# invokermyself/ICP-4DRadar

Hardware: AMD Instinct MI355X
Metric: scan-pair registrations/sec (8k-pt clouds, 20 ICP iters) at 1/2/4/8 GPU (higher is better)
Workload: dtype fp32; 1 GPU; C3/C4: 1024 independent pairs per GPU, 8192/8192-pt scans, 20 ICP iterations (fixed) + fitness pass, exact NN (kd-block pruned), PCL numerics (bit-exact float restatement); pairs_per_gpu=1024, points=8192, parallelism=1 GPU

## Files before the change

### icp-4dradar_amd/csrc/icp4r_batch.hpp

```cpp
#pragma once

#include <hip/hip_runtime.h>

#include <vector>

#include "icp4r_host.hpp"
#include "icp4r_internal.hpp"

namespace icp4r_pipe {

struct Plan {
    int q;
    bool packed;
    int splits;
    bool pruned;
    bool lds;
    bool cache;
    int leaf;
    int chunk_sb;
    int chunks;
    bool tile;
    int max_m;
    int tile_run;
    bool solo;
    int64_t blocks;
};

enum PlanOpt : int {
    kOptNnQ, kOptLeaf, kOptChunkSb, kOptNnLds, kOptNnCache, kOptNnTile, kOptTileRun, kOptSolo, kOptXpad,
    kOptPhaseTicks, kOptKd, kOptMortonMwg, kOptPart, kOptSrcOrder, kOptFuseSeed, kOptTileOwn, kOptTileDefer,
    kOptGroups, kOptSearchCuDiv, kOptFuseTest, kOptFuseOrder, kOptSumsTail, kOptWideUpdate, kOptGatherPadded,
    kOptGicpCovBrute, kOptFoldKeys, kOptGicpSpec, kOptGicpGrid, kOptGicpKnnLanes, kOptResUpdate, kOptHeldUpdate,
    kOptFitXform, kOptCounters, kOptStageSel, kOptLazyX, kNumPlanOpts
};
static_assert(kNumPlanOpts <= 64, "icp4r_ctx::plan_set is a 64-bit mask");
extern const char* const kPlanOptNames[kNumPlanOpts];
int opt(const icp4r_ctx* ctx, PlanOpt k, int dflt);

Plan make_plan(const icp4r_ctx* ctx, int npairs, int max_n, int max_m, int nn_mode = ICP4R_NN_AUTO,
               bool allow_lds = true, bool registration = false);
int make_kparams(const icp4r_params* p, icp4r::KParams* kp);
int setup_work(icp4r_ctx* ctx, const Plan& pl, int npairs, int max_n, int max_m, bool corr, hipStream_t st,
               icp4r::WorkArgs& w);
int nn_pass(icp4r_ctx* ctx, const Plan& pl, const icp4r::PairArgs& a, const icp4r::WorkArgs& w, int npairs, int max_n,
            int fitness_pass, int first, hipStream_t st, int ncu = 0, int test_fused = 0, int pass = -1,
            int ordered = 0, int pending = 0);
int next_event(std::vector<icp4r_host::EventPair>& v, size_t& used, icp4r_host::EventPair** out);

// ... 2 lines not shown
```

### icp-4dradar_amd/csrc/icp4r_capi.cpp

```cpp
#include <dlfcn.h>
#include <float.h>
#include <hip/hip_runtime.h>
#include <math.h>
#include <stdlib.h>
#include <string.h>

#include <algorithm>
#include <cstdarg>
#include <cstdio>
#include <string>
#include <utility>
#include <vector>

#include "icp4r/icp4r.h"
#include "icp4r_batch.hpp"
#include "icp4r_host.hpp"
#include "icp4r_internal.hpp"

using namespace icp4r;

namespace icp4r_host {

thread_local std::string g_last_error;

// ... 41 lines not shown
    return api;
}

}

using icp4r_host::DevBuf;
using icp4r_host::EventPair;
using icp4r_host::check_cloud;
using icp4r_host::fail;
using icp4r_host::pack_host;

namespace icp4r_pipe {

constexpr size_t kCountBytes = (size_t)kCountSlots * kCountStride * sizeof(uint64_t);

constexpr int kNumCounters = 8;
int read_counters(icp4r_ctx* ctx, uint64_t (&out)[kNumCounters]) {
    for (int k = 0; k < kNumCounters; ++k) out[k] = 0;
    HIP_TRY(hipSetDevice(ctx->device));
    HIP_TRY(hipDeviceSynchronize());
    if (!ctx->evals.p) return ICP4R_OK;
    std::vector<uint64_t> v((size_t)kCountSlots * kCountStride);
    HIP_TRY(hipMemcpy(v.data(), ctx->evals.p, kCountBytes, hipMemcpyDeviceToHost));
    for (int s = 0; s < kCountSlots; ++s)
        for (int k = 0; k < kNumCounters; ++k) out[k] += v[(size_t)s * kCountStride + k];
    return ICP4R_OK;
}

const char* const kPlanOptNames[kNumPlanOpts] = {
    "nn_q", "leaf", "chunk_sb", "nn_lds", "nn_cache", "nn_tile", "tile_run", "solo", "xpad",
    "phase_ticks", "kd", "morton_mwg", "part", "src_order", "fuse_seed", "tile_own", "tile_defer",
    "groups", "search_cu_div", "fuse_test", "fuse_order", "sums_tail", "wide_update", "gather_padded",
    "gicp_cov_brute", "fold_keys", "gicp_spec", "gicp_grid", "gicp_knn_lanes", "res_update",
    "held_update", "fit_xform", "counters", "stage_sel", "lazy_x"};

int opt(const icp4r_ctx* ctx, PlanOpt k, int dflt) {
    return (ctx && (ctx->plan_set >> k & 1ull)) ? ctx->plan_val[k] : dflt;
}

Plan make_plan(const icp4r_ctx* ctx, int npairs, int max_n, int max_m, int nn_mode, bool allow_lds,
               bool registration) {
    Plan pl;
    pl.pruned = nn_mode == ICP4R_NN_PRUNED || (nn_mode == ICP4R_NN_AUTO && max_m >= kPrunedMinM);
    pl.packed = false;
    pl.lds = false;
    pl.cache = false;
    pl.splits = 1;
    pl.leaf = 0;
    pl.chunk_sb = 64;
// ... 385 lines not shown
    const int iters = max_iterations > 0 ? max_iterations : 1;
    const bool fuse = pl.lds && pl.cache && pcl && opt(ctx, kOptFuseTest, 1) != 0;
    const bool ford = fuse && opt(ctx, kOptFuseOrder, 1) != 0;
    for (int g = 0; g < groups; ++g)
        wg[g].sums_tail = (fuse && a.kp.huber_delta == INFINITY && a.kp.max_d2 >= FLT_MAX && !a.kp.need_mse &&
                           opt(ctx, kOptSumsTail, 0) != 0)
                              ? 1
                              : 0;
    for (int g = 0; g < groups; ++g)
        wg[g].res_update = (fuse && pcl && mn <= kResMaxN && !wg[g].sums_tail && a.kp.huber_delta == INFINITY &&
                             a.kp.max_d2 >= FLT_MAX && opt(ctx, kOptResUpdate, kDefaultResUpdate) != 0)
                                ? 1
                                : 0;
    const bool lazy = fuse && !wg[0].sums_tail && !wg[0].res_update && opt(ctx, kOptLazyX, kDefaultLazyX) != 0;
    for (int g = 0; g < groups; ++g) wg[g].lazy_x = lazy ? 1 : 0;
    auto silent_tail = [&](int it) { return lazy && it >= 0 && it + 1 < iters && ((iters - 2 - it) & 1) != 0; };
    const bool kev = ctx->kernel_timing;
    const bool wide = pcl && !fuse && npairs <= ctx->ncu && opt(ctx, kOptWideUpdate, 1) != 0;
    for (int g = 0; g < groups; ++g)
        wg[g].held_update = (wide && mn <= kHeldMaxN && opt(ctx, kOptHeldUpdate, kDefaultHeldUpdate) != 0) ? 1 : 0;
    if (wide && pl.tile && !pl.lds && w.corr && (pl.chunks > 1 || !w.tile_own) && opt(ctx, kOptFoldKeys, 1) != 0)
        for (int g = 0; g < groups; ++g) wg[g].fold_keys = 1;
    char pass_name[48];
    for (int it = 0; it < iters; ++it) {
        snprintf(pass_name, sizeof(pass_name), "icp4r ICP pass %d", it + 1);
        icp4r_host::Range pass_range(pass_name);
        for (int g = 0; g < groups; ++g) {
            const int ncu_g = search_cu > 0 ? search_cu : ctx->ncu;
            if ((rc = nn_pass(ctx, pl, ag[g], wg[g], gn[g], mn, 0, it == 0, gs[g], search_cu, fuse && it > 0, it,
                              ford && it > 0, silent_tail(it - 1) ? 1 : 0)))
// ... 473 lines not shown
    return -1;
}
}

int icp4r_set_plan_option(icp4r_ctx* ctx, const char* name, int32_t value) {
    if (!ctx) return fail(ICP4R_E_INVALID, "ctx is NULL");
    const int k = plan_opt_index(name);
    if (k < 0) return fail(ICP4R_E_INVALID, "unknown plan option '%s'", name ? name : "(null)");
    if (k == kOptGroups && (value < 1 || value > kMaxGroups))
        return fail(ICP4R_E_INVALID,
                    "plan option groups = %d: 1..%d (a fourth pair group shares a hardware queue with the third, "
                    "and its kernels serialise)",
                    value, kMaxGroups);
    if (k == kOptXpad && (value < 0 || value > 1 << 20)) return fail(ICP4R_E_INVALID, "plan option xpad = %d", value);
    if (k == kOptSearchCuDiv && value < 0) return fail(ICP4R_E_INVALID, "plan option search_cu_div = %d", value);
    ctx->plan_val[k] = value;
    ctx->plan_set |= 1ull << k;
    return ICP4R_OK;
}

int icp4r_get_plan_option(const icp4r_ctx* ctx, const char* name, int32_t* value, int32_t* is_set) {
    if (!ctx || !value) return fail(ICP4R_E_INVALID, "NULL argument");
    const int k = plan_opt_index(name);
    if (k < 0) return fail(ICP4R_E_INVALID, "unknown plan option '%s'", name ? name : "(null)");
    const bool set = (ctx->plan_set >> k) & 1ull;
    *value = set ? ctx->plan_val[k] : INT32_MIN;
    if (!set) {
        static const int32_t dflt[kNumPlanOpts] = {
            0 , kDefaultLeaf, 0 , -1 , 1, 1, 0 ,
            -1 , 0, 0, 3, 1, kDefaultPartSize, -1 , 1, 1, 1, kDefaultGroups,
            0 , 1, 1, 0, 1, 0, 0, 1, kGicpSpec, kGicpGrid,
            0 , kDefaultResUpdate, kDefaultHeldUpdate, 1, 0, kDefaultStageSel, kDefaultLazyX};
        *value = dflt[k];
    }
    if (is_set) *is_set = set ? 1 : 0;
    return ICP4R_OK;
}

int icp4r_reset_plan_options(icp4r_ctx* ctx) {
    if (!ctx) return fail(ICP4R_E_INVALID, "ctx is NULL");
    ctx->plan_set = 0;
    return ICP4R_OK;
}

int icp4r_plan(const icp4r_ctx* ctx, int32_t npairs, int32_t max_src_n, int32_t max_tgt_n, int32_t nn_mode,
               int32_t numerics, icp4r_plan_info* out) {
    if (npairs <= 0 || max_src_n < 0 || max_tgt_n < 0 || !out) return fail(ICP4R_E_INVALID, "bad shape");
// ... 39 lines not shown

int icp4r_nn_stats(icp4r_ctx* ctx, icp4r_nn_stats_t* out) {
    if (!ctx || !out) return fail(ICP4R_E_INVALID, "NULL argument");
    uint64_t v[kNumCounters];
    int rc = read_counters(ctx, v);
    if (rc) return rc;
    memset(out, 0, sizeof(*out));
    out->evaluations = v[0];
    out->box_tests = v[1];
    out->cache_hits = v[2];
    out->cache_tested = v[3];
    out->records_written_by_test = v[4];
    out->tested_in_update = v[5];
    out->hits_in_update = v[6];
    out->second_chance_hits = v[7];
    return ICP4R_OK;
}

int icp4r__debug_ticks(icp4r_ctx* ctx, uint64_t* out, int32_t k) {
    if (!ctx || !out || k <= 0 || (size_t)k * sizeof(uint64_t) > ctx->ticks.cap) return fail(ICP4R_E_INVALID, "bad arguments");
    if (!ctx->ticks.p) return fail(ICP4R_E_INVALID, "phase ticks not enabled (plan option phase_ticks = 1)");
    HIP_TRY(hipSetDevice(ctx->device));
    HIP_TRY(hipDeviceSynchronize());
    HIP_TRY(hipMemcpy(out, ctx->ticks.p, (size_t)k * sizeof(uint64_t), hipMemcpyDeviceToHost));
    return ICP4R_OK;
}

int icp4r__test_rot_f32(icp4r_ctx* ctx, const float* sigma, float* R, int32_t k) {
    if (!ctx || !sigma || !R || k <= 0) return fail(ICP4R_E_INVALID, "bad arguments");
    HIP_TRY(hipSetDevice(ctx->device));
// ... 11 lines not shown
```

### icp-4dradar_amd/csrc/icp4r_frame.hip

```cpp
#include "icp4r_fold.hpp"

namespace icp4r {

template <int kInitWG>
__global__ __launch_bounds__(kInitWG) void init_kernel(PairArgs a, WorkArgs w) {
    __shared__ float Tg[16];
    __shared__ int ident;
    const int p = xcd_remap(blockIdx.x, gridDim.x);
    const int tid = threadIdx.x;
    const int n = a.src_n[p], m = a.tgt_n[p];
    const float4* src = a.src + a.src_off[p];
    const float4* tgt = a.tgt + a.tgt_off[p];
    PairState& st = w.state[p];
    if (tid < 16) Tg[tid] = a.guess ? a.guess[(int64_t)p * 16 + tid] : ((tid % 5 == 0) ? 1.0f : 0.0f);
    __syncthreads();
    if (tid == 0) {
        bool id = true;
        for (int k = 0; k < 16; ++k) id = id && (Tg[k] == ((k % 5 == 0) ? 1.0f : 0.0f));
        ident = id ? 1 : 0;
    }
    __syncthreads();
    constexpr int kInitPer = 4;
    float4* X = w.X + (int64_t)p * w.x_stride;
    const bool id = ident != 0;
// ... 53 lines not shown
        for (int k = tid; k < w.need_stride; k += kInitWG) gneed[k] = 0u;
    }
    if (tid == 0 && w.miss_cnt) w.miss_cnt[p] = 0;
    if (tid < 4 && p == 0 && w.plist_n) w.plist_n[tid] = 0;
    bad = __syncthreads_or(bad);
    big = __syncthreads_or(big);
    if (tid == 0) {
        mat4_identity(st.T_inc);
        st.prev_mse = DBL_MAX;
        st.similar = 0;
        st.conv_state = 0;
        st.iterations = 0;
        st.ncorr = 0;
        st.sums_ok = big ? -1 : 0;
        st.pending = 0;
        const bool too_big = n > w.x_stride || (w.leaf > 0 && m > w.t_stride);
        if (m <= 0 || bad || too_big) {
            mat4_identity(st.final_T);
            st.phase = kPhaseInvalid;
            st.status = too_big ? kStatusInvalid : m <= 0 ? kStatusEmpty : kStatusNonFinite;
        } else {
            for (int k = 0; k < 16; ++k) st.final_T[k] = Tg[k];
            st.phase = kPhaseActive;
            st.status = 0;
        }
    }
}

constexpr int kPrepWG = 256;
constexpr int kPrepRecs = 1024;
// ... 227 lines not shown
```

### icp-4dradar_amd/csrc/icp4r_internal.hpp

```cpp
#pragma once

#include <hip/hip_runtime.h>
#include <stdint.h>

#include "icp4r/icp4r.h"
#include "icp4r/icp4r_ego.h"
#include "icp4r/icp4r_gicp.h"
#include "icp4r_math.hpp"

namespace icp4r {

constexpr int kNNWG = 256;
constexpr int kMaxQ = 16;
constexpr int kDefaultQ = 4;
constexpr int kDefaultPrunedQ = 2;
constexpr int kDefaultLeaf = 16;
constexpr int kMaxGroups = 3;
constexpr int kDefaultGroups = 2;
constexpr int kDefaultStageSel = 32;
constexpr int kDefaultPartSize = 2048;
constexpr int kFoldChunk = 1024;
constexpr int kSuper = 8;
constexpr int kPrunedMinM = 512;
constexpr int kCacheMaxN = 16384;
// ... 29 lines not shown
};

struct PairArgs {
    const float4* src;
    const float4* tgt;
    const int64_t* src_off;
    const int32_t* src_n;
    const int64_t* tgt_off;
    const int32_t* tgt_n;
    const float* guess;
    float4* aligned;
    Result* results;
    KParams kp;
};

struct PairState {
    float T_inc[16];
    float final_T[16];
    double prev_mse;
    int32_t similar;
    int32_t conv_state;
    int32_t iterations;
    int32_t phase;
    int32_t status;
    int32_t ncorr;
    float sum_s[3];
    int32_t sums_ok;
    float T_pend[16];
    int32_t pending;
};

using NNKey = uint64_t;
__host__ __device__ inline float key_d2(NNKey k) {
    union {
        uint32_t u;
        float f;
    } c;
    c.u = (uint32_t)(k >> 32);
    return c.f;
}
__host__ __device__ inline int32_t key_idx(NNKey k) { return (int32_t)(uint32_t)k; }

struct WorkArgs {
    float4* X;
// ... 15 lines not shown
    int32_t* tinv;
    float4* tbox;
    float4* sbox;
    int32_t* sperm;
    int64_t t_stride, b_stride, sb_stride;
    float4* corr;
    float* nn_u;
    int32_t tile_own;
    int32_t defer_xform;
    int32_t sums_tail;
    int32_t fold_keys;
    int32_t res_update;
    int32_t held_update;
    int32_t fit_xform;
    int32_t lazy_x;
    float4* nn_t;
    float4* sq;
    uint2* sm;
    float4* qv;
    uint2* qm;
    uint32_t* need;
    int64_t need_stride;
    int32_t* miss_cnt;
    int32_t* plist;
    int32_t* plist_n;
    int32_t* queue;
    int32_t* owork;
    int32_t part_size;
    int32_t stage_sel;
    unsigned long long* evals;
// ... 13 lines not shown
                            int max_n, int fitness_pass, int first, hipStream_t st);
hipError_t launch_nn_tile(const PairArgs& a, const WorkArgs& w, int npairs, int max_n, int max_m, int fitness_pass,
                          int first, int qrun, hipStream_t st, hipEvent_t tile_start = nullptr, hipEvent_t tile_stop = nullptr);
struct NNLdsEvents {
    hipEvent_t test_start = nullptr, test_stop = nullptr, search_start = nullptr, search_stop = nullptr;
};
hipError_t launch_nn_lds(const PairArgs& a, const WorkArgs& w, int npairs, int max_n, int fitness_pass, int first,
                         int ncu, hipStream_t st, const NNLdsEvents& ev, int test_fused = 0, int ordered = 0,
                         int pending = 0);
constexpr int kLdsMaxTargets = 8192;
constexpr int kLdsMinPairs = 256;
constexpr int kLdsMaxSources = 1 << 14;
constexpr int kResMaxN = 8192;
constexpr int kDefaultResUpdate = 0;
constexpr int kDefaultLazyX = 1;
constexpr int kHeldMaxN = 10 * 896;
constexpr int kHeldSmallN = 3 * 704;
constexpr int kDefaultHeldUpdate = 1;
constexpr int kSoloMaxN = 1024;
hipError_t launch_update(const PairArgs& a, const WorkArgs& w, int npairs, int max_n, bool need_corr,
                         hipStream_t st, int tail_test = 0,
                         int order_ncu = 0,
                         bool wide = false,
                         int silent = 0,
                         int pending = 0);
hipError_t launch_solo(const PairArgs& a, const WorkArgs& w, int npairs, int max_n, int iters, hipStream_t st);
hipError_t launch_fitness_prep(const PairArgs& a, const WorkArgs& w, int npairs, hipStream_t st, int test = 0);
hipError_t launch_finish(const PairArgs& a, const WorkArgs& w, int npairs, hipStream_t st);
hipError_t launch_rot_f32(const float* sigma, float* R, int k, hipStream_t st);

// ... 179 lines not shown
```

### icp-4dradar_amd/csrc/icp4r_kernels.hip

```cpp
#include "icp4r_fold.hpp"

namespace icp4r {

template <int Q>
__device__ __forceinline__ void nn_sweep(const float (&x)[Q], const float (&y)[Q], const float (&z)[Q],
                                         const float4* tgt_generic, int j0, int j1, float (&best)[Q],
                                         int (&bi)[Q]) {
    const cv4f_ptr tgt = as_const(tgt_generic);
#pragma unroll
    for (int q = 0; q < Q; ++q) {
        best[q] = INFINITY;
        bi[q] = j0;
    }
    const int last = j1 - 1;
    for (int j = j0; j < j1; j += 4) {
        const v4f c[4] = {tgt[j], tgt[min(j + 1, last)], tgt[min(j + 2, last)], tgt[min(j + 3, last)]};
#pragma unroll
        for (int t = 0; t < 4; ++t) {
#pragma unroll
            for (int q = 0; q < Q; ++q) {
                const float d = l2_simple(x[q], y[q], z[q], c[t].x, c[t].y, c[t].z);
                if (d < best[q]) {
                    best[q] = d;
                    bi[q] = j + t;
// ... 1485 lines not shown
}
__device__ __forceinline__ void wave_exact_total(uint64_t& S, int& E) {
    int e = E;
#pragma unroll
    for (int off = 32; off > 0; off >>= 1) e = min(e, __shfl_xor(e, off, 64));
    uint64_t t = E == INT_MAX ? 0 : exact_rescale(S, E - e);
#pragma unroll
    for (int off = 32; off > 0; off >>= 1) t = min(t + __shfl_xor(t, off, 64), kExactSat);
    S = t;
    E = e;
}

constexpr int kSliceGroup = 14;
constexpr int kFillBatch = 2;

template <int WG, int CH, int ROW>
__device__ __forceinline__ void fold_pass_a(const KParams& kp, const FoldIn& f, float (*buf)[9][ROW], float* res,
                                            int32_t* wcnt, SolveShared& s, const float* sums = nullptr) {
    const int tid = threadIdx.x, lane = tid & 63, wave = tid >> 6;
    const bool weighted = kp.huber_delta < INFINITY;
    auto rec = [&](int i, float4& r0, float4& r1) {
        if (f.C) {
            r0 = f.C[2 * i];
            r1 = f.C[2 * i + 1];
        } else {
            r0 = f.X[i];
            r1 = f.NT[i];
        }
    };
    auto rec_fix = [&](float4& r0, float4& r1) {
        if (!f.C) {
            if (f.Tp) pend_pt(f.Tp, r0);
            const float d2 = l2_simple(r0.x, r0.y, r0.z, r1.x, r1.y, r1.z);
// ... 15 lines not shown
#pragma unroll
            for (int e = 0; e < kPerA; ++e) {
                const int i = base + min(tid - fill0 + e * nf, len - 1);
                r[e][0] = f.X[i];
                ti[e] = (uint32_t)key_idx(f.K[i]);
            }
#pragma unroll
            for (int e = 0; e < kPerA; ++e) r[e][1] = f.TG[ti[e]];
            return;
        }
#pragma unroll
        for (int e = 0; e < kPerA; ++e) {
            const int i = base + min(tid - fill0 + e * nf, len - 1);
            if (sums)
                r[e][1] = f.NT[i];
            else
                rec(i, r[e][0], r[e][1]);
        }
    };
    auto store_a = [&](int c, float4 (&r)[kPerA][2]) __attribute__((always_inline)) {
        float(*b)[ROW] = buf[c & 1];
        const int base = c * CH, len = min(CH, n - base), nf = WG - fill0;
#pragma unroll
        for (int e = 0; e < kPerA; ++e) {
            const int o = tid - fill0 + e * nf;
            if (o >= len) break;
            if (sums) {
#pragma unroll
                for (int k = 0; k < 3; ++k) b[3 + k][o] = (&r[e][1].x)[k];
                b[6][o] = 1.0f;
                ++cnt;
                continue;
            }
            rec_fix(r[e][0], r[e][1]);
            const float d2 = r[e][1].w;
            if (f.Cw) {
                f.Cw[2 * (base + o)] = r[e][0];
                f.Cw[2 * (base + o) + 1] = r[e][1];
            }
            const float sv[6] = {r[e][0].x, r[e][0].y, r[e][0].z, r[e][1].x, r[e][1].y, r[e][1].z};
            float v[6], wt = 0.0f, dd = 0.0f;
#pragma unroll
            for (int k = 0; k < 6; ++k) v[k] = ident;
            if (!(d2 > kp.max_d2)) {
                wt = r[e][0].w;
#pragma unroll
                for (int k = 0; k < 6; ++k) v[k] = weighted ? wt * sv[k] : sv[k];
                dd = d2;
                ++cnt;
            }
#pragma unroll
            for (int k = 0; k < 6; ++k) b[k][o] = v[k];
            b[6][o] = wt;
            reinterpret_cast<double*>(b[7])[o] = (double)dd;
        }
    };
    float acc = (lane < 6) ? ident : 0.0f;
    double dacc = 0.0;
    const int wv = __builtin_amdgcn_readfirstlane(wave);
    if (wv == 0) {
        const int lane0 = sums ? 3 : 0;
        fold_prio(true);
        for (int c = 0; c < nch; ++c) {
            __syncthreads();
            if (lane >= lane0 && lane < 7) acc = fold_seq<float>(buf[c & 1][lane], min(CH, n - c * CH), acc);
        }
        fold_prio(false);
    } else if (wv * 64 < fill0) {
        uint64_t xs = 0;
        int xe = INT_MAX;
        for (int c = 0; c < nch; ++c) {
            __syncthreads();
            const double* dv = reinterpret_cast<const double*>(buf[c & 1][7]);
            const int len = min(CH, n - c * CH);
            for (int o = lane; o < len; o += 64) lane_exact_add(dv[o], xs, xe);
        }
        wave_exact_total(xs, xe);
        dacc = xs >= kExactSat ? -1.0 : (xe == INT_MAX ? 0.0 : ldexp((double)xs, xe));
    } else {
        if (nch > 0) {
            float4 r[kPerA][2];
            load_a(0, r);
            store_a(0, r);
        }
        for (int c = 0; c < nch; ++c) {
            __syncthreads();
            if (c + 1 < nch) {
                float4 r[kPerA][2];
                load_a(c + 1, r);
                store_a(c + 1, r);
            }
        }
    }
    cnt = wave_sumi(cnt);
    if (lane == 0) wcnt[wave] = cnt;
    if (wave == 0 && lane < 7) res[lane] = (sums && lane < 3) ? sums[lane] : acc;
    if (wave == 1 && lane == 0) s.mse_sum = dacc;
    __syncthreads();
    if (tid == 0) {
        int total = 0;
        for (int k = 0; k < (WG / 64); ++k) total += wcnt[k];
        s.mom[0] = (double)total;
        const float one_over_n = 1.0f / res[6];
        s.one_over_n = one_over_n;
        for (int k = 0; k < 6; ++k) s.mean[k] = res[k] * one_over_n;
    }
    __syncthreads();
    if (mse && s.mse_sum < 0.0) {
        dacc = 0.0;
        if (wv == 0) {
            for (int c = 0; c < nch; ++c) __syncthreads();
        } else if (wv * 64 < fill0) {
            for (int c = 0; c < nch; ++c) {
                __syncthreads();
                if (lane == 0) dacc = fold_seq_d(reinterpret_cast<const double*>(buf[c & 1][7]), min(CH, n - c * CH), dacc);
            }
// ... 430 lines not shown
        wt[0] = __builtin_amdgcn_s_memrealtime();
        wt[5] = (uint64_t)(uint32_t)__builtin_amdgcn_s_getreg(4 | (31 << 11)) |
                ((uint64_t)(uint32_t)__builtin_amdgcn_s_getreg(20 | (31 << 11)) << 32);
    }
#define WG_TICK(k) \
    if (wt) wt[k] = __builtin_amdgcn_s_memrealtime()
#else
#define WG_TICK(k)
#endif
    const bool lazy = w.lazy_x && w.nn_u && !C && !w.sums_tail;
    const float* Tp = PEND ? st.T_pend : nullptr;
    FoldIn fin{C, Xp, NT, n};
    fin.Tp = Tp;
    const bool sums_tail = w.sums_tail && tail_test && w.nn_u && !C;
    const bool use_sums = sums_tail && uload(&st.sums_ok) == 1;
    fold_pass_a<kFoldWG, kFoldChunkP, kFoldRow>(kp, fin, sh.buf, sh.res, sh.cnt, sh.s, use_sums ? st.sum_s : nullptr);
    if (use_sums && tid == 0) st.sums_ok = 0;
    if (ticks) w.ticks[1] = __builtin_amdgcn_s_memrealtime();
    WG_TICK(1);
    fold_pass_b<kFoldWG, kFoldChunkP, kFoldRow, false>(kp, fin, sh.buf, sh.s);
    if (ticks) w.ticks[2] = __builtin_amdgcn_s_memrealtime();
    WG_TICK(2);
    const bool tail = tail_test && w.nn_u;
    int nwork = 0;
    TailFirst<kTailPer> tf;
    uint32_t* need = reinterpret_cast<uint32_t*>(&sh.buf[0][0][0]);
    if (tail) {
        if (!sums_tail && n > 0) tail_prefetch<kFoldWG, kTailPer>(w, p, n, tf);
        for (int k = tid; k < ((n + 31) >> 5); k += kFoldWG) need[k] = 0u;
        if (tid == 0) sh.mcount = 0;
    }
    if (tid == 0) solve_pair<kNumericsPCL>(sh.s, st, kp);
// ... 22 lines not shown
            float* stg = reinterpret_cast<float*>(&sh.buf[0][0][0]) + (2 * 9 * kFoldRow - 2 * kSumBuf);
            nwork = pair_cache_test<kFoldWG, kSumPer, false, true>(
                a, w, p, n, T, need, pre, lv, lm, kFoldRecsSums, &sh.mcount, sh.cnt, false, stamp, nullptr, stg,
                st.sum_s, &st.sums_ok);
        } else {
            const bool quiet = lazy && silent && !Tp;
            nwork = pair_cache_test<kFoldWG, kTailPer, false>(a, w, p, n, T, need, pre, lv, lm, kFoldRecs,
                                                                    &sh.mcount, sh.cnt, false, stamp, &tf, nullptr,
                                                                    nullptr, nullptr, Tp, quiet);
            if (quiet) {
                if (tid < 16) st.T_pend[tid] = sh.s.T_inc[tid];
                if (tid == 0) st.pending = 1;
            } else if (Tp && tid == 0) {
                st.pending = 0;
            }
        }
    }
    if (ticks) w.ticks[4] = __builtin_amdgcn_s_memrealtime();
    WG_TICK(4);
    return nwork;
}

template <bool PEND>
__global__ __launch_bounds__(kFoldWG, 4) void fold_update_kernel(PairArgs a, WorkArgs w, int tail_test, int order_ncu,
                                                                             int silent) {
    __shared__ FoldShared sh;
    __shared__ OrderShared osh;
    __shared__ int32_t last;
    const int p = xcd_remap(blockIdx.x, gridDim.x);
    const int nwork = fold_update_pair<PEND>(a, w, tail_test, silent, p, sh);
// ... 1202 lines not shown
    }
#undef ICP4R_PR_CASE
    if (chunks > 1 && w.corr != nullptr && !fitness_pass)
        hipLaunchKernelGGL(corr_kernel, dim3((max_n + 255) / 256, npairs), dim3(256), 0, st, a, w);
    return hipGetLastError();
}

hipError_t launch_update(const PairArgs& a, const WorkArgs& w, int npairs, int max_n, bool need_corr, hipStream_t st,
                         int tail_test, int order_ncu, bool wide, int silent, int pending) {
    if (silent && pending) return hipErrorInvalidValue;
    if (order_ncu > 0 && (!tail_test || !w.owork || !w.plist || !w.plist_n || !w.nn_u || a.kp.numerics != kNumericsPCL))
        return hipErrorInvalidValue;
    if (w.lazy_x && (wide || need_corr || w.corr || w.res_update || w.sums_tail || !w.nn_u || !w.defer_xform ||
                     a.kp.numerics != kNumericsPCL))
        return hipErrorInvalidValue;
    if (a.kp.numerics == kNumericsPCL) {
        if (need_corr)
            hipLaunchKernelGGL(corr_kernel, dim3((max_n + 255) / 256, npairs), dim3(256), 0, st, a, w);
        if (wide && !tail_test && order_ncu <= 0 && w.held_update && max_n <= kHeldSmallN)
            hipLaunchKernelGGL((fold_update_held_kernel<3, true>), dim3(npairs), dim3(kWideWG), 0, st, a, w);
        else if (wide && !tail_test && order_ncu <= 0 && w.held_update && max_n <= kHeldMaxN)
            hipLaunchKernelGGL((fold_update_held_kernel<10, false>), dim3(npairs), dim3(kWideWG), 0, st, a, w);
        else if (wide && !tail_test && order_ncu <= 0)
            hipLaunchKernelGGL(fold_update_wide_kernel, dim3(npairs), dim3(kWideWG), 0, st, a, w);
        else if (w.res_update && !need_corr && !w.corr && max_n <= kResMaxN && w.nn_t && w.nn_u && w.defer_xform &&
                 a.kp.huber_delta == INFINITY && a.kp.max_d2 >= FLT_MAX &&
                 !w.sums_tail && (!tail_test || (w.sq && w.sm && w.need && w.miss_cnt)))
            hipLaunchKernelGGL(fold_update_res_kernel, dim3(npairs), dim3(kResWG), 0, st, a, w, tail_test, order_ncu);
        else if (w.lazy_x && pending)
            hipLaunchKernelGGL(fold_update_kernel<true>, dim3(npairs), dim3(kFoldWG), 0, st, a, w, tail_test, order_ncu, 0);
// ... 20 lines not shown
```

### icp-4dradar_amd/icp4r/__init__.py

```python
from __future__ import annotations

import ctypes as C
import os
import sys

import numpy as np

__all__ = [
    "ICP4RError", "Params", "Result", "Batch", "Context", "IterativeClosestPoint", "library_path", "load",
    "default_params", "NUMERICS_PCL", "NUMERICS_F64", "status_name", "EXPORTED_SYMBOLS", "Comm", "shard",
    "align_batch_multi",
]

HERE = os.path.dirname(os.path.abspath(__file__))
library_path = os.environ.get("ICP4R_LIBRARY") or os.path.join(HERE, "_lib", "libicp4r.so")

OK, E_INVALID, E_EMPTY, E_TOO_FEW_CORR, E_NONFINITE, E_HIP, E_RCCL, E_NOMEM, E_TOO_LARGE = 0, -1, -2, -3, -4, -5, -6, -7, -8
NUMERICS_PCL, NUMERICS_F64 = 0, 1
NO_DEVICE = -1
NN_AUTO, NN_BRUTE, NN_BRUTE_PACKED, NN_PRUNED = 0, 1, 2, 3
STAGE_NN, STAGE_NN_TEST, STAGE_UPDATE, STAGE_BATCH, STAGE_GICP_COV = 0, 1, 2, 3, 4
DBL_MAX = sys.float_info.max

_STATUS = {OK: "ICP4R_OK", E_INVALID: "ICP4R_E_INVALID", E_EMPTY: "ICP4R_E_EMPTY",
           E_TOO_FEW_CORR: "ICP4R_E_TOO_FEW_CORR", E_NONFINITE: "ICP4R_E_NONFINITE", E_HIP: "ICP4R_E_HIP",
           E_RCCL: "ICP4R_E_RCCL", E_NOMEM: "ICP4R_E_NOMEM", E_TOO_LARGE: "ICP4R_E_TOO_LARGE"}

EXPORTED_SYMBOLS = [
    "icp4r_version", "icp4r_abi_version", "icp4r_last_error", "icp4r_params_default", "icp4r_device_count",
    "icp4r_create", "icp4r_destroy", "icp4r_align", "icp4r_align_batch_device", "icp4r_align_batch_host",
    "icp4r_fitness", "icp4r_nearest", "icp4r_synchronize", "icp4r_kernel_time_ms", "icp4r_batch_time_ms",
    "icp4r_kernel_time_reset", "icp4r_set_kernel_timing", "icp4r_plan", "icp4r_nn_counters", "icp4r_nn_cache_hits", "icp4r_stage_time_ms",
    "icp4r_nn_stats", "icp4r_set_plan_option", "icp4r_get_plan_option", "icp4r_reset_plan_options",
]
PLAN_OPTIONS = (
    "nn_q", "leaf", "chunk_sb", "nn_lds", "nn_cache", "nn_tile", "tile_run", "solo", "xpad", "phase_ticks", "kd",
    "morton_mwg", "part", "src_order", "fuse_seed", "tile_own", "tile_defer", "groups", "search_cu_div",
    "fuse_test", "fuse_order", "sums_tail", "wide_update", "gather_padded", "gicp_cov_brute", "fold_keys", "gicp_spec", "gicp_grid", "gicp_knn_lanes", "res_update", "held_update", "fit_xform", "counters", "stage_sel",
    "lazy_x",
)
EGO_EXPORTED_SYMBOLS = [
    "icp4r_ego_params_default", "icp4r_radar_features", "icp4r_ego_velocity", "icp4r_ego_velocity_batch_device",
]
GATE_EXPORTED_SYMBOLS = [
    "icp4r_compact_by_mask_batch_device", "icp4r_static_clouds_batch_device", "icp4r_static_cloud",
    "icp4r_sequence_pairs", "icp4r_register_static_sequence", "icp4r_register_static_sequence_ex",
]
GICP_EXPORTED_SYMBOLS = [
    "icp4r_gicp_params_default", "icp4r_gicp_align", "icp4r_gicp_align_batch_device", "icp4r_gicp_covariances",
]
MULTI_EXPORTED_SYMBOLS = [
    "icp4r_shard", "icp4r_align_batch_multi", "icp4r_comm_unique_id", "icp4r_comm_create", "icp4r_comm_destroy",
    "icp4r_comm_rank", "icp4r_comm_check", "icp4r_gather_results", "icp4r_align_batch_sharded",
]
# ... 107 lines not shown
        "icp4r_align_batch_host": (C.c_int, [vp, vp, vp, vp, vp, vp, vp, i32, vp, C.POINTER(Params), vp]),
        "icp4r_fitness": (C.c_int, [vp, vp, i32, i32, vp, i32, i32, vp, C.c_double, C.POINTER(C.c_double)]),
        "icp4r_nearest": (C.c_int, [vp, vp, i32, i32, vp, i32, i32, vp, vp]),
        "icp4r_synchronize": (C.c_int, [vp, vp]),
        "icp4r_kernel_time_ms": (C.c_int, [vp, C.POINTER(C.c_double), C.POINTER(i32)]),
        "icp4r_batch_time_ms": (C.c_int, [vp, C.POINTER(C.c_double), C.POINTER(i32)]),
        "icp4r_kernel_time_reset": (C.c_int, [vp]),
        "icp4r_plan": (C.c_int, [vp, i32, i32, i32, i32, i32, C.POINTER(PlanInfo)]),
        "icp4r_set_plan_option": (C.c_int, [vp, C.c_char_p, i32]),
        "icp4r_get_plan_option": (C.c_int, [vp, C.c_char_p, C.POINTER(i32), C.POINTER(i32)]),
        "icp4r_reset_plan_options": (C.c_int, [vp]),
        "icp4r_nn_counters": (C.c_int, [vp, C.POINTER(C.c_uint64), C.POINTER(C.c_uint64)]),
        "icp4r_nn_cache_hits": (C.c_int, [vp, C.POINTER(C.c_uint64)]),
        "icp4r_stage_time_ms": (C.c_int, [vp, i32, C.POINTER(C.c_double), C.POINTER(i32)]),
        "icp4r_set_kernel_timing": (C.c_int, [vp, i32]),
        "icp4r_nn_stats": (C.c_int, [vp, C.POINTER(C.c_uint64 * 8)]),
        "icp4r_map_create": (C.c_int, [vp, C.POINTER(vp)]),
        "icp4r_map_destroy": (C.c_int, [vp]),
        "icp4r_map_build": (C.c_int, [vp, vp, i64, i32]),
        "icp4r_map_add_points": (C.c_int, [vp, vp, i64, i32, i32]),
        "icp4r_map_add_scan": (C.c_int, [vp, vp, i64, i32, vp, vp, vp]),
        "icp4r_map_size": (C.c_int, [vp, C.POINTER(i64)]),
        "icp4r_map_sector_search": (C.c_int, [vp, vp, C.c_float, C.c_float, vp, i64, C.POINTER(i64)]),
        "icp4r_map_sector_search_device": (C.c_int, [vp, vp, C.c_float, C.c_float, vp, vp, vp]),
        "icp4r_map_points_device": (C.c_int, [vp, C.POINTER(vp), C.POINTER(i64)]),
        "icp4r_map_time_ms": (C.c_int, [vp, C.POINTER(C.c_double), C.POINTER(i32)]),
        "icp4r_map_time_reset": (C.c_int, [vp]),
        "icp4r_map_add_points_downsample": (C.c_int, [vp, vp, i64, i32, C.c_float, C.POINTER(i64)]),
        "icp4r_map_delete_boxes": (C.c_int, [vp, vp, i32, C.POINTER(i64)]),
        "icp4r_map_box_search": (C.c_int, [vp, vp, vp, i64, C.POINTER(i64)]),
        "icp4r_map_radius_search": (C.c_int, [vp, vp, C.c_float, vp, i64, C.POINTER(i64)]),
# ... 166 lines not shown

    def stage_time_ms(self, stage: int) -> tuple[float, int]:
        ms, k = C.c_double(), C.c_int32()
        _check(self._lib.icp4r_stage_time_ms(self._h, stage, C.byref(ms), C.byref(k)), "icp4r_stage_time_ms")
        return ms.value, k.value

    def reset_timers(self):
        _check(self._lib.icp4r_kernel_time_reset(self._h), "icp4r_kernel_time_reset")

    def nn_counters(self) -> tuple[int, int]:
        v, t = C.c_uint64(), C.c_uint64()
        _check(self._lib.icp4r_nn_counters(self._h, C.byref(v), C.byref(t)), "icp4r_nn_counters")
        return v.value, t.value

    def nn_stats(self) -> dict:
        v = (C.c_uint64 * 8)()
        _check(self._lib.icp4r_nn_stats(self._h, C.byref(v)), "icp4r_nn_stats")
        keys = ("evaluations", "box_tests", "cache_hits", "cache_tested", "records_written_by_test",
                "tested_in_update", "hits_in_update", "second_chance_hits")
        return {k: int(v[i]) for i, k in enumerate(keys)}

    def nn_cache_hits(self) -> int:
        v = C.c_uint64()
        _check(self._lib.icp4r_nn_cache_hits(self._h, C.byref(v)), "icp4r_nn_cache_hits")
        return v.value

    def nn_evaluations(self) -> int:
        return self.nn_counters()[0]


def plan(npairs: int, max_src_n: int, max_tgt_n: int, nn_mode: int = NN_AUTO, numerics: int = NUMERICS_PCL,
         ctx: "Context | None" = None) -> dict:
    info = PlanInfo()
    _check(load().icp4r_plan(ctx.handle if ctx is not None else None, npairs, max_src_n, max_tgt_n, nn_mode, numerics,
# ... 193 lines not shown
```

### include/icp4r/icp4r.h

```cpp
#ifndef ICP4R_H
#define ICP4R_H

#include <stddef.h>
#include <stdint.h>

#ifdef __cplusplus
extern "C" {
#endif

#define ICP4R_ABI_VERSION 6

typedef enum icp4r_status {
    ICP4R_OK = 0,
    ICP4R_E_INVALID = -1,
    ICP4R_E_EMPTY = -2,
    ICP4R_E_TOO_FEW_CORR = -3,
    ICP4R_E_NONFINITE = -4,
    ICP4R_E_HIP = -5,
    ICP4R_E_RCCL = -6,
    ICP4R_E_NOMEM = -7,
    ICP4R_E_TOO_LARGE = -8
} icp4r_status;

typedef enum icp4r_convergence_state {
// ... 105 lines not shown
int icp4r_stage_time_ms(icp4r_ctx* ctx, int32_t stage, double* avg_ms, int32_t* launches);

int icp4r_nn_counters(icp4r_ctx* ctx, uint64_t* evaluations, uint64_t* box_tests);

int icp4r_nn_cache_hits(icp4r_ctx* ctx, uint64_t* hits);

typedef struct icp4r_nn_stats_t {
    uint64_t evaluations;
    uint64_t box_tests;
    uint64_t cache_hits;
    uint64_t cache_tested;
    uint64_t records_written_by_test;
    uint64_t tested_in_update;
    uint64_t hits_in_update;
    uint64_t second_chance_hits;
} icp4r_nn_stats_t;
int icp4r_nn_stats(icp4r_ctx* ctx, icp4r_nn_stats_t* out);

int icp4r_set_plan_option(icp4r_ctx* ctx, const char* name, int32_t value);
int icp4r_get_plan_option(const icp4r_ctx* ctx, const char* name, int32_t* value, int32_t* is_set);
int icp4r_reset_plan_options(icp4r_ctx* ctx);

typedef struct icp4r_plan_info {
    int32_t pruned;
    int32_t q;
    int32_t splits;
    int32_t leaf;
    int32_t lds;
    int32_t cache;
    int64_t nn_blocks;
// ... 14 lines not shown
```

Before: 157,000 pairs/s.

## Carry pass-A target sums across ICP iterations when correspondences are unchanged

Adds a carry_sums mode, on by default, that caches pass A's target-side sums and correspondence count in per-pair state. On the next iteration it checks whether any of the few changed correspondences actually moved, and if none did it folds only the source coordinates and reuses the cached target sums. This skips reading and folding the gathered target points in the update kernel. It adds a validation ballot, extra per-pair state, and a subtle correctness dependency on the change-tracking records.

```diff
diff --git a/icp-4dradar_amd/csrc/icp4r_batch.hpp b/icp-4dradar_amd/csrc/icp4r_batch.hpp
--- a/icp-4dradar_amd/csrc/icp4r_batch.hpp
+++ b/icp-4dradar_amd/csrc/icp4r_batch.hpp
@@ -31,7 +31,7 @@
     kOptPhaseTicks, kOptKd, kOptMortonMwg, kOptPart, kOptSrcOrder, kOptFuseSeed, kOptTileOwn, kOptTileDefer,
     kOptGroups, kOptSearchCuDiv, kOptFuseTest, kOptFuseOrder, kOptSumsTail, kOptWideUpdate, kOptGatherPadded,
     kOptGicpCovBrute, kOptFoldKeys, kOptGicpSpec, kOptGicpGrid, kOptGicpKnnLanes, kOptResUpdate, kOptHeldUpdate,
-    kOptFitXform, kOptCounters, kOptStageSel, kOptLazyX, kNumPlanOpts
+    kOptFitXform, kOptCounters, kOptStageSel, kOptLazyX, kOptCarrySums, kNumPlanOpts
 };
 static_assert(kNumPlanOpts <= 64, "icp4r_ctx::plan_set is a 64-bit mask");
 extern const char* const kPlanOptNames[kNumPlanOpts];
diff --git a/icp-4dradar_amd/csrc/icp4r_capi.cpp b/icp-4dradar_amd/csrc/icp4r_capi.cpp
--- a/icp-4dradar_amd/csrc/icp4r_capi.cpp
+++ b/icp-4dradar_amd/csrc/icp4r_capi.cpp
@@ -79,7 +79,7 @@
 
 constexpr size_t kCountBytes = (size_t)kCountSlots * kCountStride * sizeof(uint64_t);
 
-constexpr int kNumCounters = 8;
+constexpr int kNumCounters = 10;
 int read_counters(icp4r_ctx* ctx, uint64_t (&out)[kNumCounters]) {
     for (int k = 0; k < kNumCounters; ++k) out[k] = 0;
     HIP_TRY(hipSetDevice(ctx->device));
@@ -97,7 +97,7 @@
     "phase_ticks", "kd", "morton_mwg", "part", "src_order", "fuse_seed", "tile_own", "tile_defer",
     "groups", "search_cu_div", "fuse_test", "fuse_order", "sums_tail", "wide_update", "gather_padded",
     "gicp_cov_brute", "fold_keys", "gicp_spec", "gicp_grid", "gicp_knn_lanes", "res_update",
-    "held_update", "fit_xform", "counters", "stage_sel", "lazy_x"};
+    "held_update", "fit_xform", "counters", "stage_sel", "lazy_x", "carry_sums"};
 
 int opt(const icp4r_ctx* ctx, PlanOpt k, int dflt) {
     return (ctx && (ctx->plan_set >> k & 1ull)) ? ctx->plan_val[k] : dflt;
@@ -513,6 +513,9 @@
                                 : 0;
     const bool lazy = fuse && !wg[0].sums_tail && !wg[0].res_update && opt(ctx, kOptLazyX, kDefaultLazyX) != 0;
     for (int g = 0; g < groups; ++g) wg[g].lazy_x = lazy ? 1 : 0;
+    const bool carry = fuse && !wg[0].sums_tail && !wg[0].res_update && a.kp.huber_delta == INFINITY &&
+                       a.kp.max_d2 >= FLT_MAX && !a.kp.need_mse && opt(ctx, kOptCarrySums, kDefaultCarrySums) != 0;
+    for (int g = 0; g < groups; ++g) wg[g].carry_sums = carry ? 1 : 0;
     auto silent_tail = [&](int it) { return lazy && it >= 0 && it + 1 < iters && ((iters - 2 - it) & 1) != 0; };
     const bool kev = ctx->kernel_timing;
     const bool wide = pcl && !fuse && npairs <= ctx->ncu && opt(ctx, kOptWideUpdate, 1) != 0;
@@ -1016,6 +1019,8 @@
                     value, kMaxGroups);
     if (k == kOptXpad && (value < 0 || value > 1 << 20)) return fail(ICP4R_E_INVALID, "plan option xpad = %d", value);
     if (k == kOptSearchCuDiv && value < 0) return fail(ICP4R_E_INVALID, "plan option search_cu_div = %d", value);
+    if (k == kOptCarrySums && (value < 0 || value > 1))
+        return fail(ICP4R_E_INVALID, "plan option carry_sums = %d: 0 (off) or 1 (carry pass A's target sums)", value);
     ctx->plan_val[k] = value;
     ctx->plan_set |= 1ull << k;
     return ICP4R_OK;
@@ -1032,7 +1037,8 @@
             0 , kDefaultLeaf, 0 , -1 , 1, 1, 0 ,
             -1 , 0, 0, 3, 1, kDefaultPartSize, -1 , 1, 1, 1, kDefaultGroups,
             0 , 1, 1, 0, 1, 0, 0, 1, kGicpSpec, kGicpGrid,
-            0 , kDefaultResUpdate, kDefaultHeldUpdate, 1, 0, kDefaultStageSel, kDefaultLazyX};
+            0 , kDefaultResUpdate, kDefaultHeldUpdate, 1, 0, kDefaultStageSel, kDefaultLazyX,
+            kDefaultCarrySums};
         *value = dflt[k];
     }
     if (is_set) *is_set = set ? 1 : 0;
@@ -1102,6 +1108,8 @@
     out->tested_in_update = v[5];
     out->hits_in_update = v[6];
     out->second_chance_hits = v[7];
+    out->pass_a_carried_d = v[8];
+    out->pass_a_skipped = v[9];
     return ICP4R_OK;
 }
 
diff --git a/icp-4dradar_amd/csrc/icp4r_frame.hip b/icp-4dradar_amd/csrc/icp4r_frame.hip
--- a/icp-4dradar_amd/csrc/icp4r_frame.hip
+++ b/icp-4dradar_amd/csrc/icp4r_frame.hip
@@ -91,6 +91,7 @@
         st.ncorr = 0;
         st.sums_ok = big ? -1 : 0;
         st.pending = 0;
+        st.carry.mc = -1;
         const bool too_big = n > w.x_stride || (w.leaf > 0 && m > w.t_stride);
         if (m <= 0 || bad || too_big) {
             mat4_identity(st.final_T);
diff --git a/icp-4dradar_amd/csrc/icp4r_internal.hpp b/icp-4dradar_amd/csrc/icp4r_internal.hpp
--- a/icp-4dradar_amd/csrc/icp4r_internal.hpp
+++ b/icp-4dradar_amd/csrc/icp4r_internal.hpp
@@ -67,6 +67,12 @@
     KParams kp;
 };
 
+struct CarriedSums {
+    float sum_d[4];
+    int32_t cnt;
+    int32_t mc;
+};
+
 struct PairState {
     float T_inc[16];
     float final_T[16];
@@ -81,6 +87,7 @@
     int32_t sums_ok;
     float T_pend[16];
     int32_t pending;
+    CarriedSums carry;
 };
 
 using NNKey = uint64_t;
@@ -126,6 +133,7 @@
     int32_t held_update;
     int32_t fit_xform;
     int32_t lazy_x;
+    int32_t carry_sums;
     float4* nn_t;
     float4* sq;
     uint2* sm;
@@ -169,6 +177,7 @@
 constexpr int kResMaxN = 8192;
 constexpr int kDefaultResUpdate = 0;
 constexpr int kDefaultLazyX = 1;
+constexpr int kDefaultCarrySums = 1;
 constexpr int kHeldMaxN = 10 * 896;
 constexpr int kHeldSmallN = 3 * 704;
 constexpr int kDefaultHeldUpdate = 1;
diff --git a/icp-4dradar_amd/csrc/icp4r_kernels.hip b/icp-4dradar_amd/csrc/icp4r_kernels.hip
--- a/icp-4dradar_amd/csrc/icp4r_kernels.hip
+++ b/icp-4dradar_amd/csrc/icp4r_kernels.hip
@@ -1523,9 +1523,11 @@
 constexpr int kSliceGroup = 14;
 constexpr int kFillBatch = 2;
 
-template <int WG, int CH, int ROW>
+template <int WG, int CH, int ROW, bool CARRY = false>
 __device__ __forceinline__ void fold_pass_a(const KParams& kp, const FoldIn& f, float (*buf)[9][ROW], float* res,
-                                            int32_t* wcnt, SolveShared& s, const float* sums = nullptr) {
+                                            int32_t* wcnt, SolveShared& s, const float* sums = nullptr,
+                                            const CarriedSums* cs = nullptr) {
+    constexpr bool carry = CARRY;
     const int tid = threadIdx.x, lane = tid & 63, wave = tid >> 6;
     const bool weighted = kp.huber_delta < INFINITY;
     auto rec = [&](int i, float4& r0, float4& r1) {
@@ -1571,6 +1573,8 @@
             const int i = base + min(tid - fill0 + e * nf, len - 1);
             if (sums)
                 r[e][1] = f.NT[i];
+            else if (carry)
+                r[e][0] = f.X[i];
             else
                 rec(i, r[e][0], r[e][1]);
         }
@@ -1587,6 +1591,12 @@
                 for (int k = 0; k < 3; ++k) b[3 + k][o] = (&r[e][1].x)[k];
                 b[6][o] = 1.0f;
                 ++cnt;
+                continue;
+            }
+            if (carry) {
+                if (f.Tp) pend_pt(f.Tp, r[e][0]);
+#pragma unroll
+                for (int k = 0; k < 3; ++k) b[k][o] = (&r[e][0].x)[k];
                 continue;
             }
             rec_fix(r[e][0], r[e][1]);
@@ -1616,11 +1626,11 @@
     double dacc = 0.0;
     const int wv = __builtin_amdgcn_readfirstlane(wave);
     if (wv == 0) {
-        const int lane0 = sums ? 3 : 0;
+        const int lane0 = sums ? 3 : 0, lane1 = carry ? 3 : 7;
         fold_prio(true);
         for (int c = 0; c < nch; ++c) {
             __syncthreads();
-            if (lane >= lane0 && lane < 7) acc = fold_seq<float>(buf[c & 1][lane], min(CH, n - c * CH), acc);
+            if (lane >= lane0 && lane < lane1) acc = fold_seq<float>(buf[c & 1][lane], min(CH, n - c * CH), acc);
         }
         fold_prio(false);
     } else if (wv * 64 < fill0) {
@@ -1651,12 +1661,13 @@
     }
     cnt = wave_sumi(cnt);
     if (lane == 0) wcnt[wave] = cnt;
-    if (wave == 0 && lane < 7) res[lane] = (sums && lane < 3) ? sums[lane] : acc;
+    if (wave == 0 && lane < 7) res[lane] = (sums && lane < 3) ? sums[lane] : (carry && lane >= 3) ? cs->sum_d[lane - 3] : acc;
     if (wave == 1 && lane == 0) s.mse_sum = dacc;
     __syncthreads();
     if (tid == 0) {
         int total = 0;
         for (int k = 0; k < (WG / 64); ++k) total += wcnt[k];
+        if (carry) total = cs->cnt;
         s.mom[0] = (double)total;
         const float one_over_n = 1.0f / res[6];
         s.one_over_n = one_over_n;
@@ -2117,8 +2128,38 @@
     fin.Tp = Tp;
     const bool sums_tail = w.sums_tail && tail_test && w.nn_u && !C;
     const bool use_sums = sums_tail && uload(&st.sums_ok) == 1;
-    fold_pass_a<kFoldWG, kFoldChunkP, kFoldRow>(kp, fin, sh.buf, sh.res, sh.cnt, sh.s, use_sums ? st.sum_s : nullptr);
+    bool carry = false;
+    if (w.carry_sums && w.nn_u && !C) {
+        const int mc = uload(&st.carry.mc);
+        if (mc == 0) {
+            carry = true;
+        } else if (mc > 0 && mc <= kFoldWG) {
+            bool changed = false;
+            if (tid < mc) {
+                const uint2 m = w.qm[(int64_t)p * xs + tid];
+                const int i = min((int)(m.x & kNtIdxMask), n - 1);
+                changed = nt_tpos(NT[i].w) != m.y;
+            }
+            const bool any = __ballot(changed) != 0;
+            if ((tid & 63) == 0) sh.cnt[tid >> 6] = any ? 1 : 0;
+            __syncthreads();
+            int all = 0;
+            for (int k = 0; k < kFoldWaves; ++k) all |= sh.cnt[k];
+            carry = __builtin_amdgcn_readfirstlane(all) == 0;
+        }
+        if (carry && tid == 0) count_add(w.evals, 8, 1ull);
+    }
+    if (carry)
+        fold_pass_a<kFoldWG, kFoldChunkP, kFoldRow, true>(kp, fin, sh.buf, sh.res, sh.cnt, sh.s, nullptr, &st.carry);
+    else
+        fold_pass_a<kFoldWG, kFoldChunkP, kFoldRow>(kp, fin, sh.buf, sh.res, sh.cnt, sh.s, use_sums ? st.sum_s : nullptr);
     if (use_sums && tid == 0) st.sums_ok = 0;
+    if (w.carry_sums && tid == 0) {
+#pragma unroll
+        for (int k = 0; k < 4; ++k) st.carry.sum_d[k] = sh.res[3 + k];
+        st.carry.cnt = (int32_t)sh.s.mom[0];
+        st.carry.mc = -1;
+    }
     if (ticks) w.ticks[1] = __builtin_amdgcn_s_memrealtime();
     WG_TICK(1);
     fold_pass_b<kFoldWG, kFoldChunkP, kFoldRow, false>(kp, fin, sh.buf, sh.s);
@@ -2171,6 +2212,7 @@
             } else if (Tp && tid == 0) {
                 st.pending = 0;
             }
+            if (w.carry_sums && tid == 0 && uload(&st.sums_ok) != -1) st.carry.mc = nwork <= kFoldRecs ? nwork : -1;
         }
     }
     if (ticks) w.ticks[4] = __builtin_amdgcn_s_memrealtime();
@@ -3403,6 +3445,10 @@
     if (w.lazy_x && (wide || need_corr || w.corr || w.res_update || w.sums_tail || !w.nn_u || !w.defer_xform ||
                      a.kp.numerics != kNumericsPCL))
         return hipErrorInvalidValue;
+    if (w.carry_sums && (wide || need_corr || w.corr || w.res_update || w.sums_tail || !w.nn_u || !w.nn_t || !w.qm ||
+                         a.kp.numerics != kNumericsPCL || a.kp.huber_delta != INFINITY || !(a.kp.max_d2 >= FLT_MAX) ||
+                         a.kp.need_mse))
+        return hipErrorInvalidValue;
     if (a.kp.numerics == kNumericsPCL) {
         if (need_corr)
             hipLaunchKernelGGL(corr_kernel, dim3((max_n + 255) / 256, npairs), dim3(256), 0, st, a, w);
diff --git a/icp-4dradar_amd/icp4r/__init__.py b/icp-4dradar_amd/icp4r/__init__.py
--- a/icp-4dradar_amd/icp4r/__init__.py
+++ b/icp-4dradar_amd/icp4r/__init__.py
@@ -37,7 +37,7 @@
     "nn_q", "leaf", "chunk_sb", "nn_lds", "nn_cache", "nn_tile", "tile_run", "solo", "xpad", "phase_ticks", "kd",
     "morton_mwg", "part", "src_order", "fuse_seed", "tile_own", "tile_defer", "groups", "search_cu_div",
     "fuse_test", "fuse_order", "sums_tail", "wide_update", "gather_padded", "gicp_cov_brute", "fold_keys", "gicp_spec", "gicp_grid", "gicp_knn_lanes", "res_update", "held_update", "fit_xform", "counters", "stage_sel",
-    "lazy_x",
+    "lazy_x", "carry_sums",
 )
 EGO_EXPORTED_SYMBOLS = [
     "icp4r_ego_params_default", "icp4r_radar_features", "icp4r_ego_velocity", "icp4r_ego_velocity_batch_device",
@@ -175,7 +175,7 @@
         "icp4r_nn_cache_hits": (C.c_int, [vp, C.POINTER(C.c_uint64)]),
         "icp4r_stage_time_ms": (C.c_int, [vp, i32, C.POINTER(C.c_double), C.POINTER(i32)]),
         "icp4r_set_kernel_timing": (C.c_int, [vp, i32]),
-        "icp4r_nn_stats": (C.c_int, [vp, C.POINTER(C.c_uint64 * 8)]),
+        "icp4r_nn_stats": (C.c_int, [vp, C.POINTER(C.c_uint64 * 10)]),
         "icp4r_map_create": (C.c_int, [vp, C.POINTER(vp)]),
         "icp4r_map_destroy": (C.c_int, [vp]),
         "icp4r_map_build": (C.c_int, [vp, vp, i64, i32]),
@@ -372,10 +372,10 @@
         return v.value, t.value
 
     def nn_stats(self) -> dict:
-        v = (C.c_uint64 * 8)()
+        v = (C.c_uint64 * 10)()
         _check(self._lib.icp4r_nn_stats(self._h, C.byref(v)), "icp4r_nn_stats")
         keys = ("evaluations", "box_tests", "cache_hits", "cache_tested", "records_written_by_test",
-                "tested_in_update", "hits_in_update", "second_chance_hits")
+                "tested_in_update", "hits_in_update", "second_chance_hits", "pass_a_carried_d", "pass_a_skipped")
         return {k: int(v[i]) for i, k in enumerate(keys)}
 
     def nn_cache_hits(self) -> int:
diff --git a/include/icp4r/icp4r.h b/include/icp4r/icp4r.h
--- a/include/icp4r/icp4r.h
+++ b/include/icp4r/icp4r.h
@@ -143,6 +143,8 @@
     uint64_t tested_in_update;
     uint64_t hits_in_update;
     uint64_t second_chance_hits;
+    uint64_t pass_a_carried_d;
+    uint64_t pass_a_skipped;
 } icp4r_nn_stats_t;
 int icp4r_nn_stats(icp4r_ctx* ctx, icp4r_nn_stats_t* out);
 
```

After: 159,000 pairs/s, median of 6. 1.3% higher.
